# yoyololicon/pytorch-NMF

Hardware: AMD Instinct MI355X
Metric: MU GFLOP/s (algorithmic 8*N*C*R per iteration), dense NMF 4096x65536 rank-128 beta=1; MU iterations/s alongside (higher is better)
Workload: dtype f16; 1 GPU; NMF 4096x65536 rank=128 beta=1 (BASELINE configs[1]); preset=cfg1, rows=4096, cols_per_gpu=65536, rank=128, precision=f16, parallelism=single GPU, nsplit_h=16, nsplit_w=1, block_rows_h=256, block_rows_w=256, launch=eager launches

## Files before the change

### include/nmfmu.h

```cpp
#ifndef NMFMU_H_
#define NMFMU_H_

#include <stddef.h>
#include <stdint.h>

#ifdef __cplusplus
extern "C" {
#endif

#define NMFMU_ABI_VERSION 9

#define NMFMU_OK 0
#define NMFMU_ERR_UNSUPPORTED (-2)
#define NMFMU_ERR_ARG (-3)
#define NMFMU_ERR_ALLOC (-4)

#define NMFMU_PREC_BF16 0
#define NMFMU_PREC_BF16X3 1
#define NMFMU_PREC_F16 2
#define NMFMU_PREC_F16X 3
#define NMFMU_PREC_F16R 4

#define NMFMU_BETA_KL 0
#define NMFMU_BETA_EUC 1
#define NMFMU_BETA_IS 2
#define NMFMU_BETA_GEN 3

#define NMFMU_STAGE_REG 0
#define NMFMU_STAGE_DMA 1
#define NMFMU_STAGE_DMA_NOP2 3
#define NMFMU_STAGE_DMA_LDSTR 4
#define NMFMU_STAGE_DMA_SPLIT 2

typedef struct nmfmu_factor {
  float* f;
  void* p1_hi;
  void* p1_lo;
  void* p2_hi;
  void* p2_lo;
  float* colsum;
  float* colsum_part;
  int32_t rows;
  int32_t rows_pad;
} nmfmu_factor;

typedef struct nmfmu_step {
  const void* xp;
  nmfmu_factor owner;
  nmfmu_factor panel;
  float* slab_num;
  float* slab_den;
  int32_t rank;
  int32_t r_pad;
  int32_t nsplit;
  int32_t precision;
  int32_t stage;
  int32_t block_rows;
  float beta;
  float gamma;
  float l1, l2;
  uint32_t* status;
  void* stamps;
} nmfmu_step;

int nmfmu_abi_version(void);
// ... 301 lines not shown
```

### pytorch-nmf_amd/csrc/nmfmu_capi.hip

```cpp
#include <hip/hip_runtime.h>
#include <stdint.h>

#include <algorithm>
#include <cstdlib>
#include <new>
#include <vector>

#include "../../include/nmfmu.h"
#include "nmfmu_aux.h"
#include "nmfmu_fused.h"
#include "nmfmu_pp.h"
#include "nmfmu_sp.h"
#include "nmfmu_sp2.h"

#ifndef NMFMU_SP
#define NMFMU_SP 1
#endif
#ifndef NMFMU_SP2
#define NMFMU_SP2 1
#endif
#ifndef NMFMU_FUSE_APPLY_TWO_ACC
#define NMFMU_FUSE_APPLY_TWO_ACC 1
#endif

// ... 7 lines not shown
}
inline bool x_is_f32(int precision) { return precision == NMFMU_PREC_BF16X3 || precision == NMFMU_PREC_F16X; }

#ifdef NMFMU_DEBUG_HOOKS
static int env_int(const char* name, int dflt) {
  const char* v = std::getenv(name);
  return v && *v ? std::atoi(v) : dflt;
}
static void* g_pp_debug = nullptr;
#endif
#ifndef NMFMU_PP_F16R
#define NMFMU_PP_F16R 1
#endif
static bool pp_eligible(int r_pad, int precision, float beta) {
  return nmfmu_beta_kind(beta) == NMFMU_BETA_KL && r_pad <= 128 &&
         (precision == NMFMU_PREC_F16 || precision == NMFMU_PREC_BF16 || (NMFMU_PP_F16R && precision == NMFMU_PREC_F16R));
}
static bool pp_ldstr_eligible(int r_pad, int precision, float beta) {
  return pp_eligible(r_pad, precision, beta) && pp_trl_available(r_pad, is_f16(precision) ? kOpF16 : kOpBf16, kModeMU);
}
static bool sp_eligible(int r_pad, int precision, float beta) {
  return NMFMU_SP && nmfmu_beta_kind(beta) == NMFMU_BETA_KL && r_pad == 256 && precision == NMFMU_PREC_F16;
}
static bool sp2_eligible(int r_pad, int precision, float beta) {
  const int k = nmfmu_beta_kind(beta);
  return NMFMU_SP2 && (k == NMFMU_BETA_IS || k == NMFMU_BETA_GEN) && r_pad == 128 && precision == NMFMU_PREC_F16;
}
static int kernel_beta_kind(float beta) {
  if (beta == 0.5f) return kSqrt;
  if (beta == 1.5f) return kSqrt3;
  return nmfmu_beta_kind(beta);
}

struct GramRef {
  const float* gram;
  const void* hi;
  const void* lo;
  const float* scale;
};

int fused_dispatch(const nmfmu_step* st, int mode, float* loss_part, int M, int K, hipStream_t s,
                   const float* fuse_kl_den = nullptr, bool fuse_apply = false, const GramRef* gm = nullptr) {
  if (!st || !st->owner.p1_hi || !st->panel.p1_hi) return NMFMU_ERR_ARG;
  if (!st->xp && (mode == kModeMU || mode == kModeXB)) return NMFMU_ERR_ARG;
  if (st->owner.rows_pad % kRowPad || st->panel.rows_pad % kRowPad) return NMFMU_ERR_ARG;
  if (st->block_rows != 128 && st->block_rows != 256) return NMFMU_ERR_ARG;
  if (st->stage != NMFMU_STAGE_DMA && st->stage != NMFMU_STAGE_DMA_SPLIT && st->stage != NMFMU_STAGE_DMA_NOP2 &&
      st->stage != NMFMU_STAGE_DMA_LDSTR)
    return NMFMU_ERR_UNSUPPORTED;
  const bool ldstr = st->stage == NMFMU_STAGE_DMA_LDSTR && mode != kModeLoss;
  if (ldstr && (mode != kModeMU || st->block_rows != 256 || !pp_ldstr_eligible(st->r_pad, st->precision, st->beta)))
    return NMFMU_ERR_UNSUPPORTED;
  if (st->stage == NMFMU_STAGE_DMA_SPLIT && mode == kModeMU && !(st->precision == NMFMU_PREC_BF16X3)) {
    if (nmfmu_beta_kind(st->beta) != NMFMU_BETA_KL || st->block_rows != 128) return NMFMU_ERR_UNSUPPORTED;
    mode = kModeMU2;
  }
  if (st->r_pad != pad_rank(st->rank) || st->nsplit < 1) return NMFMU_ERR_ARG;
  const bool x3 = st->precision == NMFMU_PREC_BF16X3;
  if (x3 && (!st->owner.p1_lo || !st->panel.p1_lo)) return NMFMU_ERR_ARG;
  const int kind = nmfmu_beta_kind(st->beta);
  if (st->precision == NMFMU_PREC_F16R && kind == NMFMU_BETA_EUC) return NMFMU_ERR_UNSUPPORTED;
  FusedArgs a{};
  a.xp = st->xp;
  a.p1_hi = static_cast<const uint16_t*>(st->panel.p1_hi);
  a.p1_lo = static_cast<const uint16_t*>(st->panel.p1_lo);
  a.p2_hi = static_cast<const uint16_t*>(st->panel.p2_hi);
  a.p2_lo = static_cast<const uint16_t*>(st->panel.p2_lo);
  a.a1_hi = static_cast<const uint16_t*>(st->owner.p1_hi);
  a.a1_lo = static_cast<const uint16_t*>(st->owner.p1_lo);
  a.slab_num = st->slab_num;
  a.slab_den = st->slab_den;
  a.loss_part = loss_part;
  a.M = M;
  a.K = K;
  a.M_pad = st->owner.rows_pad;
  a.ktiles = st->panel.rows_pad / kBK;
  a.nsplit = st->nsplit;
  a.tiles_per_split = (a.ktiles + st->nsplit - 1) / st->nsplit;
  a.beta = st->beta;
  a.status = st->status;
  a.cs_owner = st->owner.colsum;
  a.cs_panel = st->panel.colsum;
  if (fuse_apply) {
    a.fuse_apply = 1;
    a.rank = st->rank;
    a.f = st->owner.f;
// ... 2 lines not shown
    a.o2_hi = static_cast<uint16_t*>(st->owner.p2_hi), a.o2_lo = static_cast<uint16_t*>(st->owner.p2_lo);
    a.colsum_part = st->owner.colsum_part;
    a.l1 = st->l1, a.l2 = st->l2, a.gamma = st->gamma;
  }
  if (mode == kModeMU2) {
    if (!a.slab_num || !a.p2_hi || fuse_apply) return NMFMU_ERR_ARG;
  } else if (mode == kModeXB) {
    if (kind != kEuc || x3 || st->block_rows != 128) return NMFMU_ERR_UNSUPPORTED;
    if (!a.p2_hi || (!fuse_apply && !a.slab_num)) return NMFMU_ERR_ARG;
    if (fuse_apply && (!gm || st->r_pad > 128)) return NMFMU_ERR_ARG;
    if (gm) {
      if (!gm->hi || !gm->lo || !gm->scale || (!fuse_apply && !a.slab_den)) return NMFMU_ERR_ARG;
      a.gram_hi = static_cast<const uint16_t*>(gm->hi), a.gram_lo = static_cast<const uint16_t*>(gm->lo);
      a.gram_scale = gm->scale;
    } else {
      a.slab_den = nullptr;
    }
  } else if (mode == kModeMU || mode == kModeDen) {
    if (!a.slab_num || !a.p2_hi || (x3 && !a.p2_lo)) return NMFMU_ERR_ARG;
    if (mode == kModeMU && kind != kKL && !a.slab_den) return NMFMU_ERR_ARG;
    if (mode == kModeDen && (kind != kGen || st->block_rows != 128)) return NMFMU_ERR_UNSUPPORTED;
  } else if (!loss_part) {
    return NMFMU_ERR_ARG;
  }
  const int grid = (st->owner.rows_pad / st->block_rows) * st->nsplit;
  if (st->block_rows == 256) {
    if (!st->xp || mode == kModeDen || !pp_eligible(st->r_pad, st->precision, st->beta)) return NMFMU_ERR_UNSUPPORTED;
    a.tiles_per_split = (a.tiles_per_split + 1) & ~1;
    a.debug = mode == kModeMU ? st->stamps : nullptr;
#ifdef NMFMU_DEBUG_HOOKS
    if (mode == kModeMU && g_pp_debug) a.debug = g_pp_debug;
#endif
    if (ldstr) a.o2_hi = nullptr;
    return launch_pp(st->r_pad, is_f16(st->precision) ? kOpF16 : kOpBf16, mode, a, grid, s, st->precision == NMFMU_PREC_F16R,
                      mode == kModeMU && loss_part != nullptr, ldstr);
  }
  if (mode == kModeMU && sp_eligible(st->r_pad, st->precision, st->beta)) {
    a.tiles_per_split = (a.tiles_per_split + 3) & ~3;
    a.debug = st->stamps;
#ifdef NMFMU_DEBUG_HOOKS
    if (g_pp_debug) a.debug = g_pp_debug;
#endif
    if (st->stage == NMFMU_STAGE_DMA_NOP2) a.o2_hi = nullptr;
    return launch_sp(st->r_pad, kOpF16, a, grid, s);
  }
  if (mode == kModeMU && sp2_eligible(st->r_pad, st->precision, st->beta)) {
    a.tiles_per_split = (a.tiles_per_split + 3) & ~3;
    return launch_sp2(st->r_pad, kernel_beta_kind(st->beta), a, grid, s);
  }
  const int kk = kernel_beta_kind(st->beta);
#ifdef NMFMU_DEBUG_HOOKS
  a.debug = mode == kModeXB ? g_pp_debug : nullptr;
#endif
  switch (st->r_pad) {
    case 32: return launch_fused_r32(kk, st->precision, mode, a, grid, s);
    case 64: return launch_fused_r64(kk, st->precision, mode, a, grid, s);
    case 128: return launch_fused_r128(kk, st->precision, mode, a, grid, s);
    case 256: return launch_fused_r256(kk, st->precision, mode, a, grid, s);
  }
  return NMFMU_ERR_UNSUPPORTED;
}

struct Timer {
  std::vector<hipEvent_t> ev;
};

}

extern "C" {

int nmfmu_abi_version(void) { return NMFMU_ABI_VERSION; }
int nmfmu_abi_check(int compiled_against) { return compiled_against == NMFMU_ABI_VERSION ? NMFMU_OK : NMFMU_ERR_ARG; }
int nmfmu_pad_rows(int rows) { return rows <= 0 ? NMFMU_ERR_ARG : pad_rows(rows); }
int nmfmu_pad_rank(int rank) {
  const int r = pad_rank(rank);
  return r < 0 ? NMFMU_ERR_UNSUPPORTED : r;
// ... 91 lines not shown
  a.rows = fac->rows, a.rank = rank, a.rows_pad = fac->rows_pad;
  a.gamma = 1.f;
  a.scale = scale;
  a.skip_colsum = scale != nullptr;
  a.f16 = is_f16(precision);
  return launch_apply(r_pad, a, x3, true, S(stream));
}

int nmfmu_pack_factor(const nmfmu_factor* fac, int rank, int r_pad, int precision, void* stream) {
  return pack_factor_common(fac, rank, r_pad, precision, nullptr, stream);
}

int nmfmu_pack_factor_scaled(const nmfmu_factor* fac, int rank, int r_pad, int precision, const float* scale,
                             void* stream) {
  if (!scale) return NMFMU_ERR_ARG;
  return pack_factor_common(fac, rank, r_pad, precision, scale, stream);
}

int nmfmu_mu_partial(const nmfmu_step* st, void* stream) {
  if (!st) return NMFMU_ERR_ARG;
  if (!nmfmu_supported(st->r_pad, st->precision)) return NMFMU_ERR_UNSUPPORTED;
  return fused_dispatch(st, kModeMU, nullptr, st->owner.rows, st->panel.rows, S(stream));
}

int nmfmu_den_partial(const nmfmu_step* st, void* stream) {
  if (!st) return NMFMU_ERR_ARG;
  if (!nmfmu_supported(st->r_pad, st->precision)) return NMFMU_ERR_UNSUPPORTED;
  return fused_dispatch(st, kModeDen, nullptr, st->owner.rows, st->panel.rows, S(stream));
}

int nmfmu_mu_step(const nmfmu_step* st, const float* kl_den, int phase, void* stream) {
  if (!st || phase < 0 || phase > 2) return NMFMU_ERR_ARG;
  if (!nmfmu_supported(st->r_pad, st->precision)) return NMFMU_ERR_UNSUPPORTED;
  if (st->stage == NMFMU_STAGE_DMA_SPLIT) return NMFMU_ERR_ARG;
  const bool kl = nmfmu_beta_kind(st->beta) == NMFMU_BETA_KL;
  if (kl && !kl_den) return NMFMU_ERR_ARG;
  const bool fuse = st->nsplit == 1 && st->owner.f && st->owner.p2_hi && st->owner.colsum && st->owner.colsum_part &&
                    (kl || (NMFMU_FUSE_APPLY_TWO_ACC && st->precision != NMFMU_PREC_BF16X3 && st->r_pad <= 128));
  int e = 0;
  if (phase != 2) {
    e = fuse ? fused_dispatch(st, kModeMU, nullptr, st->owner.rows, st->panel.rows, S(stream), kl_den, true)
             : nmfmu_mu_partial(st, stream);
    if (e) return e;
  }
  if (phase != 1) {
    e = fuse ? launch_colsum_finalize(st->owner.colsum_part, st->owner.rows_pad / st->block_rows, st->r_pad,
                                      st->owner.colsum, S(stream))
             : nmfmu_mu_apply(st, nullptr, nullptr, 0, kl ? kl_den : nullptr, stream);
  }
  return e;
}

int nmfmu_colsum_nparts(const nmfmu_step* st) {
  if (!st || (st->block_rows != 128 && st->block_rows != 256)) return NMFMU_ERR_ARG;
  return st->nsplit == 1 ? st->owner.rows_pad / st->block_rows : st->owner.rows_pad / apply_stripe_rows(st->owner.rows_pad);
}

int nmfmu_pack_nparts(int rows_pad) { return rows_pad <= 0 ? NMFMU_ERR_ARG : rows_pad / apply_stripe_rows(rows_pad); }

int nmfmu_colsum_finalize(const nmfmu_factor* fac, int nparts, int r_pad, void* stream) {
  if (!fac || !fac->colsum || !fac->colsum_part || nparts <= 0) return NMFMU_ERR_ARG;
  return launch_colsum_finalize(fac->colsum_part, nparts, r_pad, fac->colsum, S(stream));
}

int nmfmu_slab_reduce(const nmfmu_step* st, float* num_out, float* den_out, void* stream) {
  if (!st || !num_out || !st->slab_num) return NMFMU_ERR_ARG;
  const int64_t plane = (int64_t)st->owner.rows_pad * st->r_pad;
  int e = launch_slab_reduce(st->slab_num, st->nsplit, plane, num_out, S(stream));
  if (e) return e;
  if (den_out) {
    if (!st->slab_den) return NMFMU_ERR_ARG;
    e = launch_slab_reduce(st->slab_den, st->nsplit, plane, den_out, S(stream));
  }
  return e;
}

static int apply_common(const nmfmu_step* st, const float* num, const float* den, int nslab, const float* kl_den,
                        int trainer, float ortho, float* grad, void* stream, int den_nslab = 0, int skip_colsum = 0) {
  if (!st || !st->owner.f) return NMFMU_ERR_ARG;
  const bool kl = nmfmu_beta_kind(st->beta) == NMFMU_BETA_KL;
  ApplyArgs a{};
  a.f = st->owner.f;
  a.num = num ? num : st->slab_num;
  a.den = num ? den : st->slab_den;
  a.nslab = num ? nslab : st->nsplit;
  a.kl_den = kl ? kl_den : nullptr;
  if (!a.num || a.nslab < 1) return NMFMU_ERR_ARG;
  a.den_nslab = den_nslab;
  a.skip_colsum = skip_colsum;
  if (kl ? !a.kl_den : !a.den) return NMFMU_ERR_ARG;
  a.p1_hi = st->owner.p1_hi, a.p1_lo = st->owner.p1_lo, a.p2_hi = st->owner.p2_hi, a.p2_lo = st->owner.p2_lo;
  a.colsum_part = st->owner.colsum_part, a.colsum = st->owner.colsum;
  a.rows = st->owner.rows, a.rank = st->rank, a.rows_pad = st->owner.rows_pad;
  a.l1 = st->l1, a.l2 = st->l2, a.gamma = st->gamma;
  a.trainer = trainer, a.ortho = ortho, a.grad = grad;
  a.f16 = is_f16(st->precision);
  a.status = st->status;
  if (!a.p1_hi || !a.p2_hi || !a.colsum || !a.colsum_part) return NMFMU_ERR_ARG;
  if (st->stage == NMFMU_STAGE_DMA_NOP2 && sp_eligible(st->r_pad, st->precision, st->beta)) a.p2_hi = a.p2_lo = nullptr;
  if (st->stage == NMFMU_STAGE_DMA_LDSTR) {
    if (st->block_rows != 256 || !pp_ldstr_eligible(st->r_pad, st->precision, st->beta)) return NMFMU_ERR_UNSUPPORTED;
    a.p2_hi = a.p2_lo = nullptr;
  }
  return launch_apply(st->r_pad, a, st->precision == NMFMU_PREC_BF16X3, false, S(stream));
}

int nmfmu_mu_apply(const nmfmu_step* st, const float* num, const float* den, int nslab, const float* kl_den,
                   void* stream) {
  return apply_common(st, num, den, nslab, kl_den, 0, 0.f, nullptr, stream);
}

int nmfmu_trainer_apply(const nmfmu_step* st, const float* num, const float* den, int nslab, const float* kl_den,
                        float ortho, float* grad, void* stream) {
  if (!(ortho >= 0.f)) return NMFMU_ERR_ARG;
  return apply_common(st, num, den, nslab, kl_den, 1, ortho, grad, stream);
}

int nmfmu_xb_supported(int r_pad, int precision, float beta) {
  if (nmfmu_beta_kind(beta) != NMFMU_BETA_EUC) return 0;
  if (r_pad != 32 && r_pad != 64 && r_pad != 128 && r_pad != 256) return 0;
  if (precision == NMFMU_PREC_F16X) return r_pad <= 128;
  return precision == NMFMU_PREC_BF16 || precision == NMFMU_PREC_F16;
}

int nmfmu_xb_partial(const nmfmu_step* st, void* stream) {
  if (!st) return NMFMU_ERR_ARG;
  if (!nmfmu_xb_supported(st->r_pad, st->precision, st->beta)) return NMFMU_ERR_UNSUPPORTED;
  return fused_dispatch(st, kModeXB, nullptr, st->owner.rows, st->panel.rows, S(stream));
}

int nmfmu_xb_step(const nmfmu_step* st, const void* g_hi, const void* g_lo, const float* g_scale, int phase, void* stream) {
  if (!st || !g_hi || !g_lo || !g_scale || phase < 0 || phase > 2) return NMFMU_ERR_ARG;
  if (!nmfmu_xb_supported(st->r_pad, st->precision, st->beta)) return NMFMU_ERR_UNSUPPORTED;
// ... 26 lines not shown
    if (he != hipSuccess) return (int)he;
  }
  e = nmfmu_comm_allreduce_sum_f32(comm, xbuf, plane + tail, stream);
  if (e) return e;
  return kl ? nmfmu_mu_apply(st, xbuf, nullptr, 1, xbuf + plane, stream)
            : nmfmu_mu_apply(st, xbuf, xbuf + plane, 1, nullptr, stream);
}

int nmfmu_loss_part_count(int owner_rows_pad, int block_rows, int nsplit) {
  if (block_rows != 128 && block_rows != 256) return NMFMU_ERR_ARG;
  return (owner_rows_pad / block_rows) * nsplit;
}

int nmfmu_loss(const nmfmu_step* st, float* loss_part, double* out, void* stream) {
  if (!st || !out) return NMFMU_ERR_ARG;
  if (!nmfmu_supported(st->r_pad, st->precision)) return NMFMU_ERR_UNSUPPORTED;
  int e = fused_dispatch(st, kModeLoss, loss_part, st->owner.rows, st->panel.rows, S(stream));
  if (e) return e;
  return launch_sum_finalize_f32(loss_part, (st->owner.rows_pad / st->block_rows) * st->nsplit, out, S(stream));
}

int nmfmu_loss_checkpoint(const nmfmu_step* st, float* loss_part, double* out2, const float* fa, float* fa_snap, int64_t na,
                          const float* fb, float* fb_snap, int64_t nb, void* stream) {
  if (!st || !loss_part || !out2 || !fa || !fa_snap || !fb || !fb_snap || na < 0 || nb < 0 || (na & 3) || (nb & 3)) return NMFMU_ERR_ARG;
  if (!nmfmu_supported(st->r_pad, st->precision)) return NMFMU_ERR_UNSUPPORTED;
  int e = fused_dispatch(st, kModeLoss, loss_part, st->owner.rows, st->panel.rows, S(stream));
  if (e) return e;
  return launch_checkpoint(loss_part, (st->owner.rows_pad / st->block_rows) * st->nsplit, st->status, out2, fa, fa_snap, na, fb,
                           fb_snap, nb, S(stream));
}

int nmfmu_riding_loss_supported(const nmfmu_step* st) {
  if (!st || !st->xp || st->block_rows != 256 || !pp_eligible(st->r_pad, st->precision, st->beta) || !is_f16(st->precision)) return 0;
  if (st->stage == NMFMU_STAGE_DMA_SPLIT || st->nsplit < 1 || !st->slab_num) return 0;
  return st->owner.f && st->owner.colsum ? 1 : 0;
}
int nmfmu_riding_loss_part_count(const nmfmu_step* st) {
  return nmfmu_riding_loss_supported(st) ? 16 * (st->owner.rows_pad / st->block_rows) * st->nsplit : NMFMU_ERR_UNSUPPORTED;
}
int nmfmu_target_sums_nparts(void) { return 1024; }
int nmfmu_target_sums(const float* v, int64_t ld, int rows, int cols, double* part, double* out4, void* stream) {
  if (!v || !part || !out4 || rows <= 0 || cols <= 0 || ld < cols) return NMFMU_ERR_ARG;
  return launch_target_sums(v, ld, rows, cols, part, nmfmu_target_sums_nparts(), out4, S(stream));
}
int nmfmu_mu_step_with_loss(const nmfmu_step* st, const float* kl_den, float* xlogs_part, const double* target_sums,
                            double* out2, void* stream) {
  if (!st || !kl_den || !xlogs_part || !target_sums || !out2) return NMFMU_ERR_ARG;
  if (!nmfmu_riding_loss_supported(st)) return NMFMU_ERR_UNSUPPORTED;
  const bool fuse = st->nsplit == 1 && st->owner.p2_hi && st->owner.colsum_part;
  int e = fuse ? fused_dispatch(st, kModeMU, xlogs_part, st->owner.rows, st->panel.rows, S(stream), kl_den, true)
               : fused_dispatch(st, kModeMU, xlogs_part, st->owner.rows, st->panel.rows, S(stream));
  if (e) return e;
  e = fuse ? launch_colsum_finalize(st->owner.colsum_part, st->owner.rows_pad / st->block_rows, st->r_pad, st->owner.colsum, S(stream))
           : nmfmu_mu_apply(st, nullptr, nullptr, 0, kl_den, stream);
  if (e) return e;
  return launch_riding_finish(xlogs_part, nmfmu_riding_loss_part_count(st) / 2, target_sums,
                              (double)st->owner.rows_pad * (double)st->panel.rows_pad, st->status, out2, S(stream));
}

int nmfmu_beta_div(const float* x, const float* y, int64_t n, float beta, double* part, double* out, void* stream) {
  if (!x || !y || !part || !out || n < 0) return NMFMU_ERR_ARG;
  return launch_beta_div(x, y, n, beta, nmfmu_beta_kind(beta), part, out, S(stream));
}

int nmfmu_mu_terms(const float* s, const float* v, int64_t n, float beta, float* gn, float* gp, void* stream) {
  if (!s || !v || !gn || !gp || n <= 0) return NMFMU_ERR_ARG;
  return launch_mu_terms(s, v, n, beta, nmfmu_beta_kind(beta), gn, gp, S(stream));
// ... 155 lines not shown
```

### pytorch-nmf_amd/csrc/nmfmu_fused.h

```cpp
#pragma once
#include <hip/hip_runtime.h>
#include <stdint.h>

#include <type_traits>

#include "nmfmu_launch.h"
#include "nmfmu_layout.h"

#ifndef NMFMU_FUSED_G1_ASM
#define NMFMU_FUSED_G1_ASM 1
#endif
#ifndef NMFMU_FUSED_TR_MINR
#define NMFMU_FUSED_TR_MINR 32
#endif


namespace nmfmu {

constexpr float kEps = 1.1920928955078125e-07f;

enum BetaKind : int { kKL = 0, kEuc = 1, kIS = 2, kGen = 3, kSqrt = 4, kSqrt3 = 5 };
enum FusedMode : int { kModeMU = 0, kModeLoss = 1, kModeDen = 2, kModeXB = 3, kModeMU2 = 4 };
enum Precision : int { kPrecBf16 = 0, kPrecX3 = 1, kPrecF16 = 2, kPrecF16X = 3, kPrecF16R = 4 };

// ... 12 lines not shown
}

struct FusedArgs {
  const void* xp;
  const uint16_t* p1_hi;
  const uint16_t* p1_lo;
  const uint16_t* p2_hi;
  const uint16_t* p2_lo;
  const uint16_t* a1_hi;
  const uint16_t* a1_lo;
  float* slab_num;
  float* slab_den;
  float* loss_part;
  int M, K;
  int M_pad, ktiles, nsplit, tiles_per_split;
  float beta;
  int fuse_apply;
  int rank;
  float* f;
  const float* kl_den;
  uint16_t* o1_hi;
  uint16_t* o1_lo;
  uint16_t* o2_hi;
  uint16_t* o2_lo;
  float* colsum_part;
  float l1, l2, gamma;
  const float* cs_owner;
  const float* cs_panel;
  const uint16_t* gram_hi;
  const uint16_t* gram_lo;
  const float* gram_scale;
  uint32_t* status;
  void* debug;
};

template <int R_PAD, int BETA, int PREC, int MODE>
struct FusedCfg {
  static constexpr bool X3 = PREC == kPrecX3;
  static constexpr bool F16 = PREC == kPrecF16 || PREC == kPrecF16X || PREC == kPrecF16R;
  static constexpr bool XR = PREC == kPrecF16R;
  static constexpr bool XF32 = X3 || PREC == kPrecF16X;
  static constexpr int BM = 128, WAVES = 4, THREADS = 256;
  static constexpr int KS = R_PAD / 16;
  static constexpr int RT = R_PAD / 32;
  static constexpr int ROWB = 2 * R_PAD;
  static constexpr int IMG = kBK * ROWB;
  static constexpr int NPL = X3 ? 2 : 1;
  static constexpr bool LOSS = MODE == kModeLoss;
  static constexpr bool DEN = MODE == kModeDen;
  static constexpr bool XB = MODE == kModeXB;
  static constexpr bool TR = R_PAD >= NMFMU_FUSED_TR_MINR && !X3 && MODE == kModeMU &&
                             (R_PAD < 256 || BETA == kKL);
  static constexpr int NIMG = ((LOSS || XB || TR) ? 1 : 2) * NPL;
  static constexpr int P1HI = 0;
  static constexpr int P1LO = IMG;
  static constexpr int P2HI = XB ? 0 : NPL * IMG;
  static constexpr int P2LO = P2HI + IMG;
  static constexpr int STAGE_BYTES = NIMG * IMG;
  static constexpr int NQ = XF32 ? 8 : (XR ? 6 : 4);
  static constexpr bool TWO_ACC = (BETA != kKL) && !LOSS && !DEN;
  static constexpr bool XSPLIT = PREC == kPrecF16X && BETA == kEuc && !LOSS && !DEN;
  static constexpr bool GNLO = X3 || XSPLIT;
  static constexpr int PASSES = IMG / 4096;
  static constexpr bool SCALE = F16 && !LOSS && (BETA == kIS || BETA == kGen || BETA == kSqrt);
  static constexpr bool DEEP = XB;
  static constexpr int MINW = XB ? (R_PAD <= 128 ? 2 : 1) : ((X3 || TWO_ACC || R_PAD > 128) ? 1 : 2);
// ... 910 lines not shown
```

### pytorch-nmf_amd/csrc/nmfmu_pp.h

```cpp
#pragma once
#include "nmfmu_fused.h"

#ifndef NMFMU_PP_DUP
#define NMFMU_PP_DUP 0
#endif
#ifndef NMFMU_PP_XM
#define NMFMU_PP_XM -1
#endif

namespace nmfmu {

template <int R_PAD, int OPT, int MODE, bool XR_ = false, bool LACC_ = false, bool TRL_ = false>
struct PPCfg {
  static constexpr int BM = 256, WAVES = 8, THREADS = 512;
  static constexpr int KS = R_PAD / 16;
  static constexpr int RT = R_PAD / 32;
  static constexpr int ROWB = 2 * R_PAD;
  static constexpr int IMG = kBK * ROWB;
  static constexpr bool LOSS = MODE == kModeLoss;
  static constexpr int LEAD = 2;
  static constexpr int NSLOT = 3;
  static constexpr bool XR = XR_;
  static constexpr int NX = XR ? 6 : 4;
  static constexpr int XTILE = BM * kBK * (XR ? 3 : 2);
  static_assert(!XR || OPT == kOpF16, "the 3-byte target comes with fp16 operands");
  static constexpr bool LACC = LACC_;
  static_assert(!LACC || (OPT == kOpF16 && MODE == kModeMU), "riding loss: fp16 operands, MU half-step");
  static constexpr bool TRL = TRL_;
  static_assert(!TRL || (MODE == kModeMU && R_PAD == 128), "transpose in LDS: MU half-step at padded rank 128");
  static constexpr bool XM = (NMFMU_PP_DUP & (4 | 32)) ? false : (NMFMU_PP_XM < 0 ? XR : NMFMU_PP_XM != 0);
  static constexpr int P1_BASE = 0, P2_BASE = NSLOT * IMG;
  static constexpr int LDS_MAIN = 2 * NSLOT * IMG;
  static constexpr int LDS_EPI = LOSS ? 64 : WAVES * 32 * R_PAD * 4;
  static constexpr int LDS_BYTES = LDS_MAIN > LDS_EPI ? LDS_MAIN : LDS_EPI;
  static constexpr int NPIECE = IMG / 1024;
  static constexpr int ND = (NPIECE + 3) / 4;
  static constexpr int NSTEP1 = 2 * KS, NSTEP2 = LOSS ? 0 : 4 * RT;
  static constexpr int PF = 4;
  static constexpr bool SCALED = OPT == kOpBf16;
  static_assert(NSTEP1 >= PF, "ring deeper than G1");
};

template <int R_PAD, int OPT, int MODE, bool XR = false, bool LACC = false, bool TRL = false>
__global__ void __launch_bounds__(512, 2) pp_kernel(const FusedArgs a) {
  using C = PPCfg<R_PAD, OPT, MODE, XR, LACC, TRL>;
  constexpr int NX = C::NX;
  constexpr int KS = C::KS, RT = C::RT, ROWB = C::ROWB, IMG = C::IMG, PF = C::PF;
  constexpr int NSTEP1 = C::NSTEP1, NSTEP2 = C::NSTEP2;
  extern __shared__ __attribute__((aligned(16))) char smem[];

  const int tid = threadIdx.x;
  const int lane = tid & 63;
  const int wave = __builtin_amdgcn_readfirstlane(tid >> 6);
  const int half = wave >> 2;
  const int j = lane & 31;
  const int hl = lane >> 5;
  const int mb = blockIdx.x / a.nsplit;
  const int ks = blockIdx.x - mb * a.nsplit;
  const int t0 = ks * a.tiles_per_split;
  const int t1 = min(t0 + a.tiles_per_split, a.ktiles);
  const int nt = t1 - t0;
  const int m0 = mb * C::BM + wave * 32 + j;

  if constexpr (OPT == kOpF16) asm volatile("s_setreg_imm32_b32 hwreg(HW_REG_MODE, 23, 1), 1");
  auto stamp = [&](int slot) {
    if constexpr (MODE == kModeMU) {
      unsigned long long* dbg = reinterpret_cast<unsigned long long*>(a.debug);
      if (!dbg) return;
      if (blockIdx.x == 0 && (wave & 3) == 0) {
        const unsigned long long c = __builtin_amdgcn_s_memtime();
        const unsigned long long r = __builtin_amdgcn_s_memrealtime();
        if (lane == 0) {
          dbg[(half * 4 + slot) * 4 + 0] = c;
          dbg[(half * 4 + slot) * 4 + 1] = r;
// ... 568 lines not shown
  }
  __syncthreads();
  if constexpr (C::LACC) {
    float lsum = (la[0] + la[1]) + (la[2] + la[3]), ssum = (ls[0] + ls[1]) + (ls[2] + ls[3]);
#pragma unroll
    for (int o = 32; o > 0; o >>= 1) lsum += __shfl_xor(lsum, o, 64), ssum += __shfl_xor(ssum, o, 64);
    if (lane == 0) a.loss_part[16 * blockIdx.x + 2 * wave] = lsum, a.loss_part[16 * blockIdx.x + 2 * wave + 1] = ssum;
  }

  int tid_e = tid;
  asm volatile("" : "+v"(tid_e));
  const int lane_e = tid_e & 63, j_e = lane_e & 31, hl_e = lane_e >> 5;
  if constexpr (C::LOSS) {
#pragma unroll
    for (int o = 32; o > 0; o >>= 1) lacc += __shfl_xor(lacc, o, 64);
    float* red = reinterpret_cast<float*>(smem);
    if (lane_e == 0) red[wave] = lacc;
    __syncthreads();
    if (tid_e == 0)
      a.loss_part[blockIdx.x] = ((red[0] + red[1]) + (red[2] + red[3])) + ((red[4] + red[5]) + (red[6] + red[7]));
  } else {
    if constexpr (SCALED) {
#pragma unroll
      for (int rt = 0; rt < RT; ++rt)
#pragma unroll
        for (int e = 0; e < 16; ++e) acc[rt][e] *= 8388608.f;
    }
    const int mrow0 = mb * C::BM + wave * 32;
    if (a.fuse_apply) {
      constexpr int LDT = R_PAD;
      constexpr int SP = R_PAD / 8;
      constexpr int NCH = (32 * SP) / 64;
      float* tile = reinterpret_cast<float*>(smem) + wave * (32 * LDT);
      const int slot_e = lane_e % SP, rl0 = lane_e / SP;
      float den8[8], csum8[8];
#pragma unroll
      for (int k = 0; k < 8; ++k) { den8[k] = a.kl_den[slot_e * 8 + k]; csum8[k] = 0.f; }
      const bool vec = (a.rank & 3) == 0;
      bool clamped = false;
      static_for<RT>([&](auto rtc) {
        constexpr int rt = decltype(rtc)::value;
#pragma unroll
        for (int e = 0; e < 16; ++e) tile[((e & 3) + 8 * (e >> 2) + 4 * hl_e) * LDT + rt * 32 + j_e] = acc[rt][e];
      });
      __syncthreads();
      const bool plain = a.l1 <= 0.f && a.l2 <= 0.f && a.gamma == 1.f && a.rank == R_PAD &&
                         mb * C::BM + C::BM <= a.M;
      if (plain) {
        float rden8[8];
#pragma unroll
        for (int k = 0; k < 8; ++k) rden8[k] = 1.f / den8[k];
#pragma unroll 4
        for (int i = 0; i < NCH; ++i) {
          const int rl = i * (64 / SP) + rl0, row = mrow0 + rl, r0 = slot_e * 8;
          float* trow = tile + rl * LDT + r0;
          float* frow = a.f + (size_t)row * R_PAD + r0;
          float fv[8], nm[8];
          *reinterpret_cast<float4*>(fv) = *reinterpret_cast<const float4*>(frow);
          *reinterpret_cast<float4*>(fv + 4) = *reinterpret_cast<const float4*>(frow + 4);
          *reinterpret_cast<float4*>(nm) = *reinterpret_cast<const float4*>(trow);
          *reinterpret_cast<float4*>(nm + 4) = *reinterpret_cast<const float4*>(trow + 4);
#pragma unroll
          for (int k = 0; k < 8; ++k) {
            fv[k] *= (fmaxf(nm[k], 0.f) + kEps) * rden8[k];
            csum8[k] += fv[k];
            if constexpr (OPT == kOpF16) clamped |= fv[k] > 65504.f;
          }
          *reinterpret_cast<float4*>(frow) = *reinterpret_cast<const float4*>(fv);
          *reinterpret_cast<float4*>(frow + 4) = *reinterpret_cast<const float4*>(fv + 4);
          *reinterpret_cast<float4*>(trow) = *reinterpret_cast<const float4*>(fv);
          *reinterpret_cast<float4*>(trow + 4) = *reinterpret_cast<const float4*>(fv + 4);
          u32x4 hi;
#pragma unroll
          for (int qq = 0; qq < 4; ++qq) hi[qq] = pack_op<OPT>(fv[2 * qq], fv[2 * qq + 1]);
          *reinterpret_cast<u32x4*>(reinterpret_cast<char*>(a.o1_hi) + p1_offset(row, r0, R_PAD)) = hi;
        }
      } else
#pragma unroll 2
      for (int i = 0; i < NCH; ++i) {
        const int rl = i * (64 / SP) + rl0, row = mrow0 + rl, r0 = slot_e * 8;
        float* trow = tile + rl * LDT + r0;
        float* frow = a.f + (size_t)row * a.rank + r0;
        float fv[8], nm[8];
        *reinterpret_cast<float4*>(nm) = *reinterpret_cast<const float4*>(trow);
        *reinterpret_cast<float4*>(nm + 4) = *reinterpret_cast<const float4*>(trow + 4);
#pragma unroll
        for (int h = 0; h < 2; ++h) {
          const bool in = row < a.M && r0 + 4 * h < a.rank;
          if (in && vec) {
            *reinterpret_cast<float4*>(fv + 4 * h) = *reinterpret_cast<const float4*>(frow + 4 * h);
          } else {
#pragma unroll
            for (int k = 0; k < 4; ++k) fv[4 * h + k] = (in && r0 + 4 * h + k < a.rank) ? frow[4 * h + k] : 0.f;
          }
        }
#pragma unroll
        for (int k = 0; k < 8; ++k) {
          const float neg = fmaxf(nm[k], 0.f) + kEps;
          float pos = den8[k];
          if (a.l1 > 0.f) pos += a.l1;
          if (a.l2 > 0.f) pos += a.l2 * fv[k];
          float mult = neg / pos;
          if (a.gamma != 1.f) mult = mu_pow(mult, a.gamma);
          fv[k] = (row < a.M && r0 + k < a.rank) ? fv[k] * mult : 0.f;
          csum8[k] += fv[k];
          if constexpr (OPT == kOpF16) clamped |= fv[k] > 65504.f;
        }
#pragma unroll
        for (int h = 0; h < 2; ++h) {
          const bool in = row < a.M && r0 + 4 * h < a.rank;
          if (in && vec) {
            *reinterpret_cast<float4*>(frow + 4 * h) = *reinterpret_cast<const float4*>(fv + 4 * h);
          } else if (in) {
#pragma unroll
            for (int k = 0; k < 4; ++k)
              if (r0 + 4 * h + k < a.rank) frow[4 * h + k] = fv[4 * h + k];
          }
        }
        *reinterpret_cast<float4*>(trow) = *reinterpret_cast<const float4*>(fv);
        *reinterpret_cast<float4*>(trow + 4) = *reinterpret_cast<const float4*>(fv + 4);
        u32x4 hi;
#pragma unroll
        for (int qq = 0; qq < 4; ++qq) hi[qq] = pack_op<OPT>(fv[2 * qq], fv[2 * qq + 1]);
        *reinterpret_cast<u32x4*>(reinterpret_cast<char*>(a.o1_hi) + p1_offset(row, r0, R_PAD)) = hi;
      }
      if constexpr (OPT == kOpF16) {
        if (a.status && __any(clamped) && lane_e == 0) atomicOr(a.status, 1u);
      }
      if (a.o2_hi) {
        __syncthreads();
#pragma unroll
        for (int ii = 0; ii < R_PAD / 64 + (R_PAD < 64 ? 1 : 0); ++ii) {
          const int r = ii * 64 + lane_e;
          if (r < R_PAD) {
#pragma unroll
            for (int g = 0; g < 4; ++g) {
              const float* src = tile + (g * 8) * LDT + r;
              u32x4 hi;
#pragma unroll
              for (int qq = 0; qq < 4; ++qq) hi[qq] = pack_op<OPT>(src[(2 * qq) * LDT], src[(2 * qq + 1) * LDT]);
              *reinterpret_cast<u32x4*>(reinterpret_cast<char*>(a.o2_hi) + p2_offset(mrow0 + g * 8, r, R_PAD)) = hi;
            }
          }
        }
      }
      __syncthreads();
      float* red = reinterpret_cast<float*>(smem);
#pragma unroll
      for (int k = 0; k < 8; ++k) {
        float tot = csum8[k];
        if constexpr (SP <= 32) tot += __shfl_xor(tot, 32, 64);
        if constexpr (SP <= 16) tot += __shfl_xor(tot, 16, 64);
        if constexpr (SP <= 8) tot += __shfl_xor(tot, 8, 64);
        if constexpr (SP <= 4) tot += __shfl_xor(tot, 4, 64);
        if (lane_e < SP) red[wave * R_PAD + slot_e * 8 + k] = tot;
      }
      __syncthreads();
      for (int r = tid_e; r < R_PAD; r += C::THREADS) {
        float tot = (red[r] + red[R_PAD + r]) + (red[2 * R_PAD + r] + red[3 * R_PAD + r]);
        tot += (red[4 * R_PAD + r] + red[5 * R_PAD + r]) + (red[6 * R_PAD + r] + red[7 * R_PAD + r]);
        a.colsum_part[(size_t)mb * R_PAD + r] = tot;
      }
    } else {
      const size_t slab = ((size_t)ks * a.M_pad + (size_t)mrow0) * R_PAD;
      static_for<RT>([&](auto rtc) {
        constexpr int rt = decltype(rtc)::value;
#pragma unroll
        for (int e = 0; e < 16; ++e) {
          const int row = (e & 3) + 8 * (e >> 2) + 4 * hl_e;
          a.slab_num[slab + (size_t)row * R_PAD + rt * 32 + j_e] = acc[rt][e];
        }
      });
    }
  }
  if constexpr (MODE == kModeMU) {
    if (a.debug) asm volatile("s_waitcnt vmcnt(0)" ::: "memory");
    stamp(3);
  }
}

template <int R_PAD, int OPT, int MODE, bool XR = false, bool LACC = false, bool TRL = false>
int launch_pp_one(const FusedArgs& a, int grid, hipStream_t s) {
  using C = PPCfg<R_PAD, OPT, MODE, XR, LACC, TRL>;
  return launch_with_dynamic_lds<pp_kernel<R_PAD, OPT, MODE, XR, LACC, TRL>, C::THREADS, C::LDS_BYTES>(dim3(grid), s, a);
}

int launch_pp(int r_pad, int opt, int mode, const FusedArgs& a, int grid, hipStream_t s, bool xr = false, bool lacc = false,
              bool trl = false);
bool pp_available(int r_pad, int opt, int mode);
bool pp_trl_available(int r_pad, int opt, int mode);

}
```

### pytorch-nmf_amd/torchnmf_amd/_capi.py

```python
from __future__ import annotations

import ctypes as C
import os
from typing import Optional

LIB_NAME = 'libnmfmu.so'
LIB_PATH = os.environ.get('NMFMU_LIB') or os.path.join(os.path.dirname(os.path.abspath(__file__)), LIB_NAME)

OK = 0
ERR_UNSUPPORTED = -2
ERR_ARG = -3
ERR_ALLOC = -4
PREC_BF16, PREC_BF16X3, PREC_F16, PREC_F16X, PREC_F16R = 0, 1, 2, 3, 4
STAGE_REG, STAGE_DMA, STAGE_DMA_SPLIT = 0, 1, 2
STAGE_DMA_NOP2 = 3
STAGE_DMA_LDSTR = 4
BETA_KL, BETA_EUC, BETA_IS, BETA_GEN = 0, 1, 2, 3
KERNEL_FUSED, KERNEL_PP, KERNEL_SP = 0, 1, 2

PRECISIONS = {'bf16': PREC_BF16, 'bf16x3': PREC_BF16X3, 'f16': PREC_F16, 'f16x': PREC_F16X, 'f16r': PREC_F16R}


class NmfmuError(RuntimeError):
    pass


class Factor(C.Structure):
    _fields_ = [('f', C.c_void_p), ('p1_hi', C.c_void_p), ('p1_lo', C.c_void_p), ('p2_hi', C.c_void_p),
                ('p2_lo', C.c_void_p), ('colsum', C.c_void_p), ('colsum_part', C.c_void_p), ('rows', C.c_int32),
                ('rows_pad', C.c_int32)]


class Step(C.Structure):
    _fields_ = [('xp', C.c_void_p), ('owner', Factor), ('panel', Factor), ('slab_num', C.c_void_p),
                ('slab_den', C.c_void_p), ('rank', C.c_int32), ('r_pad', C.c_int32), ('nsplit', C.c_int32),
                ('precision', C.c_int32), ('stage', C.c_int32), ('block_rows', C.c_int32), ('beta', C.c_float), ('gamma', C.c_float),
                ('l1', C.c_float), ('l2', C.c_float), ('status', C.c_void_p), ('stamps', C.c_void_p)]


class GemmDesc(C.Structure):
    _fields_ = [('a_hi', C.c_void_p), ('a_lo', C.c_void_p), ('b_hi', C.c_void_p), ('b_lo', C.c_void_p),
                ('m_pad', C.c_int32), ('n_pad', C.c_int32), ('k_pad', C.c_int32), ('precision', C.c_int32),
                ('beta', C.c_float), ('x', C.c_void_p), ('gn_hi', C.c_void_p), ('gn_lo', C.c_void_p),
                ('gp_hi', C.c_void_p), ('gp_lo', C.c_void_p), ('out', C.c_void_p), ('m_valid', C.c_int32),
                ('n_valid', C.c_int32), ('ops', C.c_int32), ('t_batch', C.c_int32), ('t_rank', C.c_int32),
                ('t_taps', C.c_int32), ('t_lh', C.c_int32), ('tile_rows', C.c_int32), ('n_ld', C.c_int32), ('k_len', C.c_int32), ('k_split', C.c_int32),
                ('tail_rows', C.c_int32), ('rag_c0', C.c_int32), ('rag_channels', C.c_int32),
                ('win_nd', C.c_int32), ('win_lh', C.c_int32 * 3), ('win_taps', C.c_int32 * 3), ('win_channels', C.c_int32),
                ('win_pitch', C.c_int32), ('win_fold', C.c_int32), ('t_koff', C.c_void_p), ('stage_mode', C.c_int32)]
# ... 237 lines not shown
```

### pytorch-nmf_amd/torchnmf_amd/engine.py

```python
from __future__ import annotations

import ctypes as C
import os
from typing import Optional

import torch

from . import _capi


def _ptr(t: Optional[torch.Tensor]) -> Optional[int]:
    return None if t is None else t.data_ptr()


class HipBackend:

    name = 'hip'

    def __init__(self):
        self.lib = _capi.load()
        if not torch.cuda.is_available():
            raise _capi.NmfmuError('torchnmf_amd needs a ROCm device (MI355X); none is visible and there is no '
                                   'CPU fallback')

# ... 381 lines not shown

    @classmethod
    def auto_single_plane(cls, V, W, H, r_pad, be, group=None) -> Optional[str]:
        if (os.environ.get('TORCHNMF_AMD_AUTO_F16', '1') == '0' or not hasattr(_capi, 'PREC_F16')
                or not be.supported(r_pad, _capi.PREC_F16)):
            return None
        dims_ok = min(V.shape) >= cls.F16_MIN_DIM
        if group is None and not dims_ok:
            return None
        in_range, exact = cls.f16_stats(V, W, H, be) if dims_ok else (False, False)
        level = 2 if (in_range and exact) else (1 if in_range else 0)
        if level == 1 and not (hasattr(_capi, 'PREC_F16X') and be.supported(r_pad, _capi.PREC_F16X)
                               and os.environ.get('TORCHNMF_AMD_AUTO_F16X', '1') != '0'):
            level = 0
        if group is not None:
            import torch.distributed as dist
            flag = torch.tensor([level], dtype=torch.int32, device=V.device)
            dist.all_reduce(flag, op=dist.ReduceOp.MIN, group=group)
            level = int(flag.item())
            if level == 1 and not (hasattr(_capi, 'PREC_F16X') and be.supported(r_pad, _capi.PREC_F16X)):
                level = 0
        return {2: 'f16', 1: 'f16x', 0: None}[level]

    @classmethod
    def auto_mode(cls, V, W, H, r_pad, be, beta, group=None) -> Optional[str]:
        mode = cls.auto_single_plane(V, W, H, r_pad, be, group)
        if (mode == 'f16x' and float(beta) != 2.0 and hasattr(_capi, 'PREC_F16R') and be.supported(r_pad, _capi.PREC_F16R)
                and os.environ.get('TORCHNMF_AMD_AUTO_F16R', '1') != '0'):
            mode = 'f16r'
        return mode

    def __init__(self, V, W, H, beta, l1=0.0, l2=0.0, precision='auto', stage=None, group=None, backend=None,
                 update_W=True, update_H=True, block_rows=None, allow_f16=False, ar_overlap=None, allow_gram=False,
                 ar_direct=None):
        self.be = backend if backend is not None else DEFAULT_BACKEND_FACTORY()
        self.group = group
        self.beta = float(beta)
        self.kl = self.beta == 1.0
        N, Cc = V.shape
        R = W.shape[1]
        assert W.shape == (Cc, R) and H.shape == (N, R)
        if V.stride(1) != 1 or V.dtype != torch.float32:
            V = V.float().contiguous()
        self.rank = R
        self.r_pad = self.be.pad_rank(R)
        if precision in (None, 'auto'):
            precision = self.auto_mode(V, W, H, self.r_pad, self.be, self.beta, group) if allow_f16 else None
            if precision is None:
                if not self.be.supported(self.r_pad, _capi.PREC_BF16X3):
                    raise NotImplementedError(
                        f"precision='auto' found no mode for rank {R} that meets the 1e-4 parity bar on the fused kernels "
                        f"(fp16 operands -- 'f16', or 'f16x' with an fp32 target -- need both dimensions >= {self.F16_MIN_DIM} "
                        f"and data within fp16's range; split bf16 stops at rank 128); pass precision='bf16' (factors "
                        f"~1e-3), 'f16' or 'f16x' explicitly")
                precision = 'bf16x3'
        if precision not in _capi.PRECISIONS:
            raise ValueError(f"precision must be one of {sorted(_capi.PRECISIONS)} or 'auto', got {precision!r}")
        self.precision_name = precision
        self.precision = _capi.PRECISIONS[precision]
        if not self.be.supported(self.r_pad, self.precision):
            raise NotImplementedError(f'precision {precision!r} is not available for rank {R} (padded {self.r_pad})')
        if stage is None:
            nop2 = (hasattr(self.be, 'kernel_family') and hasattr(_capi, 'STAGE_DMA_NOP2') and float(beta) == 1.0
                    and self.r_pad == 256 and self.be.kernel_family(self.r_pad, self.precision, float(beta)) == _capi.KERNEL_SP
                    and os.environ.get('TORCHNMF_AMD_NO_P2', '1') != '0')
            stage = _capi.STAGE_DMA_NOP2 if nop2 else _capi.STAGE_DMA
            if (group is None and update_W and block_rows in (None, 256) and hasattr(self.be, 'pp_lds_transpose_supported')
                    and self.be.pp_lds_transpose_supported(self.r_pad, self.precision, float(beta))
                    and self.be.block_rows(self.r_pad, self.precision, float(beta)) == 256):
                stage = _capi.STAGE_DMA_LDSTR
        self.gram_path = (allow_gram and self.beta == 2.0 and group is None and block_rows in (None, 128)
                          and hasattr(self.be, 'xb_supported') and self.be.xb_supported(self.r_pad, self.precision, self.beta)
                          and os.environ.get('TORCHNMF_AMD_BETA2_GRAM', '1') != '0')
        gamma = mu_gamma(self.beta)
        dev = V.device

        self.fW = FactorBuf(W, self.r_pad, self.precision, self.be)
        self.fH = FactorBuf(H, self.r_pad, self.precision, self.be)
        self.flags = torch.tensor([0, 0x7f800000], dtype=torch.int32, device=dev)
        self.status = torch.zeros(1, dtype=torch.int32, device=dev)
        n_pad, c_pad = self.fH.rows_pad, self.fW.rows_pad
        def tile_rows(m_pad, k_pad):
            if block_rows is not None:
                return block_rows
            if hasattr(self.be, 'step_block_rows'):
                return self.be.step_block_rows(m_pad, k_pad, self.r_pad, self.precision, self.beta, dev)
            return self.be.block_rows(self.r_pad, self.precision, self.beta)
        br = tile_rows(n_pad, c_pad)
        self.block_rows = br
        xp_h = self.be.pack_x(V, False, self.precision, br, n_pad, c_pad, self.flags)
        ns_h = self._nsplit(n_pad, c_pad, br, dev)
        need_den = False if self.kl else ('one' if self.gram_path else True)
        self.step_h = StepBuf(xp_h, self.fH, self.fW, R, self.r_pad, ns_h, self.precision, stage, br, self.beta, gamma,
                              l1, l2, need_den=need_den, status=self.status)
        self.step_w = None
        if update_W:
            brw = tile_rows(c_pad, n_pad)
            xp_w = self.be.pack_x(V, True, self.precision, brw, c_pad, n_pad, None)
            ns_w = self._nsplit(c_pad, n_pad, brw, dev)
            self.step_w = StepBuf(xp_w, self.fW, self.fH, R, self.r_pad, ns_w, self.precision, stage, brw, self.beta,
                                  gamma, l1, l2, need_den=need_den, status=self.status)
        self.gm = self.be.gram_alloc(self.r_pad, dev) if self.gram_path else None
        self.timer: Optional[KernelTimer] = None
        self.refresh_images()
        self.loss_part = torch.empty(max((n_pad // br) * ns_h, 1), dtype=torch.float32, device=dev)
        self.loss_out = torch.zeros(1, dtype=torch.float64, device=dev)
        self._riding = None
        self._riding_pending = False
        if (group is None and self.kl and self.step_w is not None and update_H and hasattr(self.be, 'riding_supported')
                and os.environ.get('TORCHNMF_AMD_RIDING_LOSS', '1') != '0' and V.dtype == torch.float32 and V.stride(1) == 1
                and self.be.riding_supported(self.step_w)):
            self._riding = {'V': V, 'bufs': None}
        if group is not None:
            tail = self.r_pad if self.kl else self.step_h.plane
            self.xbuf = torch.empty(self.step_h.plane + tail, dtype=torch.float32, device=dev)
            explicit_direct = bool(ar_direct)
            if ar_direct is None:
                ar_direct = os.environ.get('TORCHNMF_AMD_COMM', 'torch') == 'c'
            self._comm = None
            if ar_direct and hasattr(self.be, 'comm_init'):
                self._comm = self.be.comm_init(group, dev)
                ar_overlap = False
            elif explicit_direct:
                raise _capi.NmfmuError("allreduce='direct' needs the library's own RCCL communicator (nmfmu_comm_*), which "
                                       f"the {getattr(self.be, 'name', type(self.be).__name__)} backend does not provide")
            st = self.step_h
            nblk = st.owner.rows_pad // 256
            frac = float(os.environ.get('TORCHNMF_AMD_AR_SPLIT', '0.5'))
            r0 = min(max(int(frac * nblk + 1e-9), 1), max(nblk - 1, 1)) * 256
            self._h_rows = None
            if ar_overlap is None:
                ar_overlap = os.environ.get('TORCHNMF_AMD_AR_OVERLAP', '0') != '0'
            if (ar_overlap and nblk >= 2 and st.owner.rows > r0
# ... 198 lines not shown
```

Before: 898,600 GFLOP/s.

## Stage split-K slab stores through LDS with coalesced write-through stores

When a row block is split across several K partitions (nsplit_h=16 here), the partial-accumulator slab write now goes through shared memory first. Each wave stores its accumulators into an LDS tile, then copies it out as coalesced 16-byte global stores, which by default carry the sc1 cache-policy bit so the slab is written through for the later reduction. The epilogue also skips the LDS tile write-back when no second packed panel is needed, and folds the column-sum update into an FMA. This adds a __syncthreads and LDS traffic to the split path in exchange for fewer, wider global stores, and the stage field now carries a flag bit behind an environment toggle.

Result: no change. 899,400 GFLOP/s, median of 3 (+0.1%).

```diff
diff --git a/include/nmfmu.h b/include/nmfmu.h
--- a/include/nmfmu.h
+++ b/include/nmfmu.h
@@ -31,6 +31,9 @@
 #define NMFMU_STAGE_DMA_NOP2 3
 #define NMFMU_STAGE_DMA_LDSTR 4
 #define NMFMU_STAGE_DMA_SPLIT 2
+
+#define NMFMU_STAGE_KIND_MASK 0xff
+#define NMFMU_STAGE_PLAIN_STORES 0x100
 
 typedef struct nmfmu_factor {
   float* f;
diff --git a/pytorch-nmf_amd/csrc/nmfmu_capi.hip b/pytorch-nmf_amd/csrc/nmfmu_capi.hip
--- a/pytorch-nmf_amd/csrc/nmfmu_capi.hip
+++ b/pytorch-nmf_amd/csrc/nmfmu_capi.hip
@@ -63,6 +63,8 @@
   return nmfmu_beta_kind(beta);
 }
 
+static int stage_kind(const nmfmu_step* st) { return st->stage & NMFMU_STAGE_KIND_MASK; }
+
 struct GramRef {
   const float* gram;
   const void* hi;
@@ -76,13 +78,13 @@
   if (!st->xp && (mode == kModeMU || mode == kModeXB)) return NMFMU_ERR_ARG;
   if (st->owner.rows_pad % kRowPad || st->panel.rows_pad % kRowPad) return NMFMU_ERR_ARG;
   if (st->block_rows != 128 && st->block_rows != 256) return NMFMU_ERR_ARG;
-  if (st->stage != NMFMU_STAGE_DMA && st->stage != NMFMU_STAGE_DMA_SPLIT && st->stage != NMFMU_STAGE_DMA_NOP2 &&
-      st->stage != NMFMU_STAGE_DMA_LDSTR)
+  if (stage_kind(st) != NMFMU_STAGE_DMA && stage_kind(st) != NMFMU_STAGE_DMA_SPLIT && stage_kind(st) != NMFMU_STAGE_DMA_NOP2 &&
+      stage_kind(st) != NMFMU_STAGE_DMA_LDSTR)
     return NMFMU_ERR_UNSUPPORTED;
-  const bool ldstr = st->stage == NMFMU_STAGE_DMA_LDSTR && mode != kModeLoss;
+  const bool ldstr = stage_kind(st) == NMFMU_STAGE_DMA_LDSTR && mode != kModeLoss;
   if (ldstr && (mode != kModeMU || st->block_rows != 256 || !pp_ldstr_eligible(st->r_pad, st->precision, st->beta)))
     return NMFMU_ERR_UNSUPPORTED;
-  if (st->stage == NMFMU_STAGE_DMA_SPLIT && mode == kModeMU && !(st->precision == NMFMU_PREC_BF16X3)) {
+  if (stage_kind(st) == NMFMU_STAGE_DMA_SPLIT && mode == kModeMU && !(st->precision == NMFMU_PREC_BF16X3)) {
     if (nmfmu_beta_kind(st->beta) != NMFMU_BETA_KL || st->block_rows != 128) return NMFMU_ERR_UNSUPPORTED;
     mode = kModeMU2;
   }
@@ -151,6 +153,7 @@
     if (mode == kModeMU && g_pp_debug) a.debug = g_pp_debug;
 #endif
     if (ldstr) a.o2_hi = nullptr;
+    a.write_through = (st->stage & NMFMU_STAGE_PLAIN_STORES) ? 0 : 1;
     return launch_pp(st->r_pad, is_f16(st->precision) ? kOpF16 : kOpBf16, mode, a, grid, s, st->precision == NMFMU_PREC_F16R,
                       mode == kModeMU && loss_part != nullptr, ldstr);
   }
@@ -160,7 +163,7 @@
 #ifdef NMFMU_DEBUG_HOOKS
     if (g_pp_debug) a.debug = g_pp_debug;
 #endif
-    if (st->stage == NMFMU_STAGE_DMA_NOP2) a.o2_hi = nullptr;
+    if (stage_kind(st) == NMFMU_STAGE_DMA_NOP2) a.o2_hi = nullptr;
     return launch_sp(st->r_pad, kOpF16, a, grid, s);
   }
   if (mode == kModeMU && sp2_eligible(st->r_pad, st->precision, st->beta)) {
@@ -318,7 +321,7 @@
 int nmfmu_mu_step(const nmfmu_step* st, const float* kl_den, int phase, void* stream) {
   if (!st || phase < 0 || phase > 2) return NMFMU_ERR_ARG;
   if (!nmfmu_supported(st->r_pad, st->precision)) return NMFMU_ERR_UNSUPPORTED;
-  if (st->stage == NMFMU_STAGE_DMA_SPLIT) return NMFMU_ERR_ARG;
+  if (stage_kind(st) == NMFMU_STAGE_DMA_SPLIT) return NMFMU_ERR_ARG;
   const bool kl = nmfmu_beta_kind(st->beta) == NMFMU_BETA_KL;
   if (kl && !kl_den) return NMFMU_ERR_ARG;
   const bool fuse = st->nsplit == 1 && st->owner.f && st->owner.p2_hi && st->owner.colsum && st->owner.colsum_part &&
@@ -383,8 +386,8 @@
   a.f16 = is_f16(st->precision);
   a.status = st->status;
   if (!a.p1_hi || !a.p2_hi || !a.colsum || !a.colsum_part) return NMFMU_ERR_ARG;
-  if (st->stage == NMFMU_STAGE_DMA_NOP2 && sp_eligible(st->r_pad, st->precision, st->beta)) a.p2_hi = a.p2_lo = nullptr;
-  if (st->stage == NMFMU_STAGE_DMA_LDSTR) {
+  if (stage_kind(st) == NMFMU_STAGE_DMA_NOP2 && sp_eligible(st->r_pad, st->precision, st->beta)) a.p2_hi = a.p2_lo = nullptr;
+  if (stage_kind(st) == NMFMU_STAGE_DMA_LDSTR) {
     if (st->block_rows != 256 || !pp_ldstr_eligible(st->r_pad, st->precision, st->beta)) return NMFMU_ERR_UNSUPPORTED;
     a.p2_hi = a.p2_lo = nullptr;
   }
@@ -477,7 +480,7 @@
 
 int nmfmu_riding_loss_supported(const nmfmu_step* st) {
   if (!st || !st->xp || st->block_rows != 256 || !pp_eligible(st->r_pad, st->precision, st->beta) || !is_f16(st->precision)) return 0;
-  if (st->stage == NMFMU_STAGE_DMA_SPLIT || st->nsplit < 1 || !st->slab_num) return 0;
+  if (stage_kind(st) == NMFMU_STAGE_DMA_SPLIT || st->nsplit < 1 || !st->slab_num) return 0;
   return st->owner.f && st->owner.colsum ? 1 : 0;
 }
 int nmfmu_riding_loss_part_count(const nmfmu_step* st) {
diff --git a/pytorch-nmf_amd/csrc/nmfmu_fused.h b/pytorch-nmf_amd/csrc/nmfmu_fused.h
--- a/pytorch-nmf_amd/csrc/nmfmu_fused.h
+++ b/pytorch-nmf_amd/csrc/nmfmu_fused.h
@@ -68,6 +68,7 @@
   const float* gram_scale;
   uint32_t* status;
   void* debug;
+  int write_through;
 };
 
 template <int R_PAD, int BETA, int PREC, int MODE>
diff --git a/pytorch-nmf_amd/csrc/nmfmu_pp.h b/pytorch-nmf_amd/csrc/nmfmu_pp.h
--- a/pytorch-nmf_amd/csrc/nmfmu_pp.h
+++ b/pytorch-nmf_amd/csrc/nmfmu_pp.h
@@ -40,6 +40,12 @@
   static constexpr bool SCALED = OPT == kOpBf16;
   static_assert(NSTEP1 >= PF, "ring deeper than G1");
 };
+
+template <bool WT>
+__device__ __forceinline__ void epi_store16(void* p, u32x4 v) {
+  if constexpr (WT) asm volatile("global_store_dwordx4 %0, %1, off sc1\n\ts_nop 1" ::"v"(p), "v"(v));
+  else *reinterpret_cast<u32x4*>(p) = v;
+}
 
 template <int R_PAD, int OPT, int MODE, bool XR = false, bool LACC = false, bool TRL = false>
 __global__ void __launch_bounds__(512, 2) pp_kernel(const FusedArgs a) {
@@ -674,6 +680,7 @@
       constexpr int SP = R_PAD / 8;
       constexpr int NCH = (32 * SP) / 64;
       float* tile = reinterpret_cast<float*>(smem) + wave * (32 * LDT);
+      const bool keep_tile = a.o2_hi != nullptr;
       const int slot_e = lane_e % SP, rl0 = lane_e / SP;
       float den8[8], csum8[8];
 #pragma unroll
@@ -704,14 +711,17 @@
           *reinterpret_cast<float4*>(nm + 4) = *reinterpret_cast<const float4*>(trow + 4);
 #pragma unroll
           for (int k = 0; k < 8; ++k) {
-            fv[k] *= (fmaxf(nm[k], 0.f) + kEps) * rden8[k];
-            csum8[k] += fv[k];
+            const float mult = (fmaxf(nm[k], 0.f) + kEps) * rden8[k];
+            csum8[k] = __builtin_fmaf(fv[k], mult, csum8[k]);
+            fv[k] *= mult;
             if constexpr (OPT == kOpF16) clamped |= fv[k] > 65504.f;
           }
           *reinterpret_cast<float4*>(frow) = *reinterpret_cast<const float4*>(fv);
           *reinterpret_cast<float4*>(frow + 4) = *reinterpret_cast<const float4*>(fv + 4);
-          *reinterpret_cast<float4*>(trow) = *reinterpret_cast<const float4*>(fv);
-          *reinterpret_cast<float4*>(trow + 4) = *reinterpret_cast<const float4*>(fv + 4);
+          if (keep_tile) {
+            *reinterpret_cast<float4*>(trow) = *reinterpret_cast<const float4*>(fv);
+            *reinterpret_cast<float4*>(trow + 4) = *reinterpret_cast<const float4*>(fv + 4);
+          }
           u32x4 hi;
 #pragma unroll
           for (int qq = 0; qq < 4; ++qq) hi[qq] = pack_op<OPT>(fv[2 * qq], fv[2 * qq + 1]);
@@ -759,8 +769,10 @@
               if (r0 + 4 * h + k < a.rank) frow[4 * h + k] = fv[4 * h + k];
           }
         }
-        *reinterpret_cast<float4*>(trow) = *reinterpret_cast<const float4*>(fv);
-        *reinterpret_cast<float4*>(trow + 4) = *reinterpret_cast<const float4*>(fv + 4);
+        if (keep_tile) {
+          *reinterpret_cast<float4*>(trow) = *reinterpret_cast<const float4*>(fv);
+          *reinterpret_cast<float4*>(trow + 4) = *reinterpret_cast<const float4*>(fv + 4);
+        }
         u32x4 hi;
 #pragma unroll
         for (int qq = 0; qq < 4; ++qq) hi[qq] = pack_op<OPT>(fv[2 * qq], fv[2 * qq + 1]);
@@ -769,7 +781,7 @@
       if constexpr (OPT == kOpF16) {
         if (a.status && __any(clamped) && lane_e == 0) atomicOr(a.status, 1u);
       }
-      if (a.o2_hi) {
+      if (keep_tile) {
         __syncthreads();
 #pragma unroll
         for (int ii = 0; ii < R_PAD / 64 + (R_PAD < 64 ? 1 : 0); ++ii) {
@@ -804,15 +816,24 @@
         a.colsum_part[(size_t)mb * R_PAD + r] = tot;
       }
     } else {
-      const size_t slab = ((size_t)ks * a.M_pad + (size_t)mrow0) * R_PAD;
+      float* tile = reinterpret_cast<float*>(smem) + wave * (32 * R_PAD);
       static_for<RT>([&](auto rtc) {
         constexpr int rt = decltype(rtc)::value;
 #pragma unroll
-        for (int e = 0; e < 16; ++e) {
-          const int row = (e & 3) + 8 * (e >> 2) + 4 * hl_e;
-          a.slab_num[slab + (size_t)row * R_PAD + rt * 32 + j_e] = acc[rt][e];
-        }
+        for (int e = 0; e < 16; ++e) tile[((e & 3) + 8 * (e >> 2) + 4 * hl_e) * R_PAD + rt * 32 + j_e] = acc[rt][e];
       });
+      __syncthreads();
+      const size_t slab = ((size_t)ks * a.M_pad + (size_t)mrow0) * R_PAD;
+      char* dst = reinterpret_cast<char*>(a.slab_num + slab);
+      auto copy_out = [&](auto wtc) {
+#pragma unroll
+        for (int i = 0; i < (32 * R_PAD * 4) / 1024; ++i) {
+          const int off = i * 1024 + lane_e * 16;
+          epi_store16<decltype(wtc)::value>(dst + off, *reinterpret_cast<const u32x4*>(reinterpret_cast<const char*>(tile) + off));
+        }
+      };
+      if (a.write_through) copy_out(std::true_type{});
+      else copy_out(std::false_type{});
     }
   }
   if constexpr (MODE == kModeMU) {
diff --git a/pytorch-nmf_amd/torchnmf_amd/_capi.py b/pytorch-nmf_amd/torchnmf_amd/_capi.py
--- a/pytorch-nmf_amd/torchnmf_amd/_capi.py
+++ b/pytorch-nmf_amd/torchnmf_amd/_capi.py
@@ -15,6 +15,8 @@
 STAGE_REG, STAGE_DMA, STAGE_DMA_SPLIT = 0, 1, 2
 STAGE_DMA_NOP2 = 3
 STAGE_DMA_LDSTR = 4
+STAGE_KIND_MASK = 0xff
+STAGE_PLAIN_STORES = 0x100
 BETA_KL, BETA_EUC, BETA_IS, BETA_GEN = 0, 1, 2, 3
 KERNEL_FUSED, KERNEL_PP, KERNEL_SP = 0, 1, 2
 
diff --git a/pytorch-nmf_amd/torchnmf_amd/engine.py b/pytorch-nmf_amd/torchnmf_amd/engine.py
--- a/pytorch-nmf_amd/torchnmf_amd/engine.py
+++ b/pytorch-nmf_amd/torchnmf_amd/engine.py
@@ -437,7 +437,7 @@
 
     def __init__(self, V, W, H, beta, l1=0.0, l2=0.0, precision='auto', stage=None, group=None, backend=None,
                  update_W=True, update_H=True, block_rows=None, allow_f16=False, ar_overlap=None, allow_gram=False,
-                 ar_direct=None):
+                 ar_direct=None, write_through=None):
         self.be = backend if backend is not None else DEFAULT_BACKEND_FACTORY()
         self.group = group
         self.beta = float(beta)
@@ -474,6 +474,10 @@
                     and self.be.pp_lds_transpose_supported(self.r_pad, self.precision, float(beta))
                     and self.be.block_rows(self.r_pad, self.precision, float(beta)) == 256):
                 stage = _capi.STAGE_DMA_LDSTR
+        if write_through is None:
+            write_through = os.environ.get('TORCHNMF_AMD_PP_WRITE_THROUGH', '1') != '0'
+        self.write_through = bool(write_through)
+        stage_flags = 0 if self.write_through else _capi.STAGE_PLAIN_STORES
         self.gram_path = (allow_gram and self.beta == 2.0 and group is None and block_rows in (None, 128)
                           and hasattr(self.be, 'xb_supported') and self.be.xb_supported(self.r_pad, self.precision, self.beta)
                           and os.environ.get('TORCHNMF_AMD_BETA2_GRAM', '1') != '0')
@@ -496,14 +500,14 @@
         xp_h = self.be.pack_x(V, False, self.precision, br, n_pad, c_pad, self.flags)
         ns_h = self._nsplit(n_pad, c_pad, br, dev)
         need_den = False if self.kl else ('one' if self.gram_path else True)
-        self.step_h = StepBuf(xp_h, self.fH, self.fW, R, self.r_pad, ns_h, self.precision, stage, br, self.beta, gamma,
+        self.step_h = StepBuf(xp_h, self.fH, self.fW, R, self.r_pad, ns_h, self.precision, stage | stage_flags, br, self.beta, gamma,
                               l1, l2, need_den=need_den, status=self.status)
         self.step_w = None
         if update_W:
             brw = tile_rows(c_pad, n_pad)
             xp_w = self.be.pack_x(V, True, self.precision, brw, c_pad, n_pad, None)
             ns_w = self._nsplit(c_pad, n_pad, brw, dev)
-            self.step_w = StepBuf(xp_w, self.fW, self.fH, R, self.r_pad, ns_w, self.precision, stage, brw, self.beta,
+            self.step_w = StepBuf(xp_w, self.fW, self.fH, R, self.r_pad, ns_w, self.precision, stage | stage_flags, brw, self.beta,
                                   gamma, l1, l2, need_den=need_den, status=self.status)
         self.gm = self.be.gram_alloc(self.r_pad, dev) if self.gram_path else None
         self.timer: Optional[KernelTimer] = None
```
